# lbrndnr/LBAudioDetective

Measured on AMD Instinct MI355X. Metric: audio_seconds_fingerprinted_per_sec, higher is better.
Workload: dtype f32; 1 GPU; configs[1]: 100k synthetic 1 s @44.1 kHz mono clips, 1024-pt FFT, stride 64, fingerprint-only, input resident in HBM; one step = 13 passes over the batch; clips_per_gpu=100000, samples_per_clip=44100, window=1024, stride=64, bands=32, subfingerprints_per_clip=5, kernel_variant=0, parallelism=clips sharded x1, no collective

## Files before the change

### include/lbaudiodetective.h

```cpp
#ifndef LBAUDIODETECTIVE_H
#define LBAUDIODETECTIVE_H

#include <stddef.h>
#include <stdint.h>

#ifdef __cplusplus
extern "C" {
#endif

#if !defined(__MACTYPES__) && !defined(LBAD_HAVE_MACTYPES)
typedef uint32_t UInt32;
typedef int32_t SInt32;
typedef uint64_t UInt64;
typedef int64_t SInt64;
typedef float Float32;
typedef double Float64;
typedef unsigned char Boolean;
typedef SInt32 OSStatus;
enum { noErr = 0 };
#endif

#if !defined(__CoreAudioTypes_h__) && !defined(LBAD_HAVE_COREAUDIOTYPES)
typedef struct AudioStreamBasicDescription {
    Float64 mSampleRate;
// ... 115 lines not shown
                                                   UInt32 inResamplerMode, Float32** outSamples, UInt64* outCount,
                                                   Float64* outSampleRate);
void LBAudioDetectiveFreeSamples(Float32* inSamples);
OSStatus LBAudioDetectiveProcessFileStream(LBAudioDetectiveRef inDetective, const Float32* inClientSamples,
                                           UInt64 inClientCount, UInt64 inFileFrames, UInt32 inHop,
                                           LBAudioDetectiveFingerprintRef* outFingerprint);

UInt64 LBAudioDetectiveGetSubfingerprintCount(LBAudioDetectiveRef inDetective, UInt64 inNumberOfSamples);

OSStatus LBAudioDetectiveProcessPCM(LBAudioDetectiveRef inDetective, const Float32* inSamples,
                                    UInt64 inNumberOfSamples, LBAudioDetectiveFingerprintRef* outFingerprint);
OSStatus LBAudioDetectiveComparePCM(LBAudioDetectiveRef inDetective, const Float32* inSamples1, UInt64 inCount1,
                                    const Float32* inSamples2, UInt64 inCount2, UInt32 inComparisonRange,
                                    Float32* outMatch);

#define LBAD_PACKED_WORDS 8
#define LBAD_PACKED_BYTES 32
#define LBAD_MAX_SUBFINGERPRINT_LENGTH 256

OSStatus LBAudioDetectiveFingerprintClipsDevice(LBAudioDetectiveRef inDetective, const Float32* inClips,
                                                UInt64 inNumberOfClips, UInt64 inSamplesPerClip,
                                                void* outPacked, void* inStream);
OSStatus LBAudioDetectiveFingerprintClipsDeviceFormat(LBAudioDetectiveRef inDetective, const void* inClips,
                                                      UInt32 inSampleFormat, UInt64 inNumberOfClips,
                                                      UInt64 inSamplesPerClip, void* outPacked, void* inStream);
OSStatus LBAudioDetectiveFingerprintClips(LBAudioDetectiveRef inDetective, const Float32* inClips,
                                          UInt64 inNumberOfClips, UInt64 inSamplesPerClip, Boolean* outBooleans);
OSStatus LBAudioDetectiveFingerprintClipsFormat(LBAudioDetectiveRef inDetective, const void* inClips,
                                                UInt32 inSampleFormat, UInt64 inNumberOfClips,
                                                UInt64 inSamplesPerClip, Boolean* outBooleans);
OSStatus LBAudioDetectiveSetKernelVariant(LBAudioDetectiveRef inDetective, UInt32 inVariant);
OSStatus LBAudioDetectiveSetBandSumForm(LBAudioDetectiveRef inDetective, UInt32 inForm);
OSStatus LBAudioDetectiveGetBandSumForm(LBAudioDetectiveRef inDetective, UInt32* outForm);
OSStatus LBAudioDetectiveSetKernelTuning(LBAudioDetectiveRef inDetective, UInt32 inWavesPerWorkgroup,
                                         UInt32 inTwiddleCache);
OSStatus LBAudioDetectiveSetScratchLimit(LBAudioDetectiveRef inDetective, UInt64 inBytes);
OSStatus LBAudioDetectiveSetStageTiming(LBAudioDetectiveRef inDetective, UInt32 inEnabled);
OSStatus LBAudioDetectiveGetStageTimes(LBAudioDetectiveRef inDetective, Float32* outStage1Ms, Float32* outStage2Ms,
                                       UInt32* outLaunches);
OSStatus LBAudioDetectiveFingerprintClipsDeviceTaps(LBAudioDetectiveRef inDetective, const Float32* inClips,
                                                    UInt64 inNumberOfClips, UInt64 inSamplesPerClip,
                                                    void* outPacked, Float32* outFramesRaw, Float32* outFramesHaar,
                                                    void* inStream);
OSStatus LBAudioDetectiveFingerprintClipsDeviceTapsFormat(LBAudioDetectiveRef inDetective, const void* inClips,
                                                          UInt32 inSampleFormat, UInt64 inNumberOfClips,
                                                          UInt64 inSamplesPerClip, void* outPacked, Float32* outFramesRaw,
                                                          Float32* outFramesHaar, void* inStream);
OSStatus LBAudioDetectiveDebugStage1Choice(Float64 inSampleRate, UInt32 inWindowSize, UInt32 inAnalysisStride,
                                           UInt32 inNumberOfPitchSteps, UInt32 inSubfingerprintLength, UInt32 inKernelVariant,
                                           UInt32 inWavesPerWorkgroup, UInt32 inTwiddleCache, UInt32 inSampleFormat,
                                           UInt64 inNumberOfClips, UInt64 inSamplesPerClip, UInt32 inClipAddressMod8,
                                           UInt32 inRawTap, UInt32 inFileTail, UInt32* outWords, UInt32 inCapacity);

typedef struct LBAudioDetectiveStream* LBAudioDetectiveStreamRef;
LBAudioDetectiveStreamRef LBAudioDetectiveStreamNew(LBAudioDetectiveRef inDetective);
void LBAudioDetectiveStreamDispose(LBAudioDetectiveStreamRef inStream);
OSStatus LBAudioDetectiveStreamPush(LBAudioDetectiveStreamRef inStream, const Float32* inSamples,
                                    UInt64 inNumberOfSamples, UInt32* outNewSubfingerprints);
LBAudioDetectiveFingerprintRef LBAudioDetectiveStreamCopyFingerprint(LBAudioDetectiveStreamRef inStream);

typedef struct LBAudioDetectiveStreamBank* LBAudioDetectiveStreamBankRef;
LBAudioDetectiveStreamBankRef LBAudioDetectiveStreamBankNew(LBAudioDetectiveRef inDetective, UInt32 inNumberOfChannels,
                                                            UInt32 inHistorySubfingerprints, UInt32 inFramesPerPass);
void LBAudioDetectiveStreamBankDispose(LBAudioDetectiveStreamBankRef inBank);
OSStatus LBAudioDetectiveStreamBankPushDevice(LBAudioDetectiveStreamBankRef inBank, const Float32* inSamples,
                                              const UInt32* inSampleCounts, UInt32* outNewCounts, void* outNewPacked,
// ... 354 lines not shown
```

### lbaudiodetective_amd/_native.py

```python
from __future__ import annotations

import ctypes as C
import os
import subprocess

_HERE = os.path.dirname(os.path.abspath(__file__))
CSRC = os.path.join(_HERE, "csrc")
LIB_PATH = os.path.abspath(os.environ["LBAD_LIB"]) if os.environ.get("LBAD_LIB") else os.path.join(_HERE, "lib", "liblbaudiodetective.so")
HEADER = os.path.join(os.path.dirname(_HERE), "include", "lbaudiodetective.h")

UInt32, SInt32, UInt64, SInt64 = C.c_uint32, C.c_int32, C.c_uint64, C.c_int64
Float32, Float64, Boolean, OSStatus = C.c_float, C.c_double, C.c_ubyte, C.c_int32
Ref = C.c_void_p

PACKED_WORDS = 8
PACKED_BYTES = 32
SHARD_KEYS = 4096
ROWS_PER_FRAME = 128
SEGMENTS_MAX_SUBFINGERPRINTS = 8192


class AudioStreamBasicDescription(C.Structure):
    _fields_ = [
        ("mSampleRate", Float64), ("mFormatID", UInt32), ("mFormatFlags", UInt32),
# ... 82 lines not shown
    "LBAudioDetectiveCompactFramesToSubfingerprintsDevice": (OSStatus, [Ref, C.c_void_p, UInt64, C.c_void_p, C.c_void_p, C.c_void_p]),
    "LBAudioDetectiveFramesToSubfingerprintsDevice": (OSStatus, [Ref, C.c_void_p, UInt64, C.c_void_p, C.c_void_p, C.c_void_p]),
    "LBAudioDetectiveStreamNew": (Ref, [Ref]),
    "LBAudioDetectiveStreamDispose": (None, [Ref]),
    "LBAudioDetectiveStreamPush": (OSStatus, [Ref, C.c_void_p, UInt64, _P(UInt32)]),
    "LBAudioDetectiveStreamCopyFingerprint": (Ref, [Ref]),
    "LBAudioDetectiveStreamBankNew": (Ref, [Ref, UInt32, UInt32, UInt32]),
    "LBAudioDetectiveStreamBankDispose": (None, [Ref]),
    "LBAudioDetectiveStreamBankPushDevice": (OSStatus, [Ref, C.c_void_p, _P(UInt32), _P(UInt32), C.c_void_p, UInt64, _P(UInt64), C.c_void_p]),
    "LBAudioDetectiveStreamBankPush": (OSStatus, [Ref, C.c_void_p, _P(UInt32), _P(UInt32), C.c_void_p, UInt64, _P(UInt64), C.c_void_p]),
    "LBAudioDetectiveStreamBankGetCounts": (OSStatus, [Ref, _P(UInt64), _P(UInt32)]),
    "LBAudioDetectiveStreamBankWindowDevice": (OSStatus, [Ref, _P(UInt32), UInt32, UInt32, C.c_void_p, C.c_void_p]),
    "LBAudioDetectiveStreamBankCopyFingerprint": (Ref, [Ref, UInt32]),
    "LBAudioDetectiveStreamBankResetChannels": (OSStatus, [Ref, _P(UInt32), UInt32]),
    "LBAudioDetectiveDebugStreamBankPlan": (OSStatus, [UInt32, UInt32, UInt32, UInt32, _P(UInt32), _P(UInt32), _P(UInt32), _P(UInt32),
                                                       _P(UInt32)]),
    "LBAudioDetectiveResamplerBankNew": (Ref, [Float64, Float64, UInt32, UInt32]),
    "LBAudioDetectiveResamplerBankDispose": (None, [Ref]),
    "LBAudioDetectiveResamplerBankPushDevice": (OSStatus, [Ref, C.c_void_p, UInt32, _P(UInt32), _P(UInt32), C.c_void_p, UInt64, _P(UInt64),
                                                           C.c_void_p]),
    "LBAudioDetectiveResamplerBankPush": (OSStatus, [Ref, C.c_void_p, UInt32, _P(UInt32), _P(UInt32), C.c_void_p, UInt64, _P(UInt64),
                                                     C.c_void_p]),
    "LBAudioDetectiveResamplerBankFinishChannels": (OSStatus, [Ref, _P(UInt32), UInt32, _P(UInt32), C.c_void_p, UInt64, _P(UInt64),
                                                               C.c_void_p]),
    "LBAudioDetectiveResamplerBankGetCounts": (OSStatus, [Ref, _P(UInt64), _P(UInt64)]),
    "LBAudioDetectiveResamplerBankResetChannels": (OSStatus, [Ref, _P(UInt32), UInt32]),
    "LBAudioDetectiveDebugResamplerBankPlan": (OSStatus, [Float64, Float64, UInt32, UInt32, _P(UInt64), _P(UInt64), _P(UInt32), UInt32,
                                                          _P(UInt32), _P(UInt32), _P(SInt32), _P(SInt32)]),
    "LBAudioDetectiveFingerprintClips": (OSStatus, [Ref, C.c_void_p, UInt64, UInt64, C.c_void_p]),
    "LBAudioDetectiveFingerprintClipsFormat": (OSStatus, [Ref, C.c_void_p, UInt32, UInt64, UInt64, C.c_void_p]),
    "LBAudioDetectiveSetKernelVariant": (OSStatus, [Ref, UInt32]),
    "LBAudioDetectiveSetBandSumForm": (OSStatus, [Ref, UInt32]),
    "LBAudioDetectiveGetBandSumForm": (OSStatus, [Ref, _P(UInt32)]),
    "LBAudioDetectiveSetScratchLimit": (OSStatus, [Ref, UInt64]),
    "LBAudioDetectiveSetStageTiming": (OSStatus, [Ref, UInt32]),
    "LBAudioDetectiveGetStageTimes": (OSStatus, [Ref, _P(Float32), _P(Float32), _P(UInt32)]),
    "LBAudioDetectiveFingerprintClipsDeviceTapsFormat": (OSStatus, [Ref, C.c_void_p, UInt32, UInt64, UInt64, C.c_void_p, C.c_void_p,
                                                                    C.c_void_p, C.c_void_p]),
    "LBAudioDetectiveDebugStage1Choice": (OSStatus, [Float64, UInt32, UInt32, UInt32, UInt32, UInt32, UInt32, UInt32, UInt32, UInt64,
                                                     UInt64, UInt32, UInt32, UInt32, _P(UInt32), UInt32]),
    "LBAudioDetectiveFingerprintClipsDeviceTaps": (OSStatus, [Ref, C.c_void_p, UInt64, UInt64, C.c_void_p, C.c_void_p,
                                                              C.c_void_p, C.c_void_p]),
    "LBAudioDetectivePackSubfingerprint": (None, [C.c_void_p, UInt32, C.c_void_p]),
    "LBAudioDetectiveUnpackSubfingerprint": (None, [C.c_void_p, UInt32, C.c_void_p]),
    "LBAudioDetectiveCorpusNew": (Ref, [UInt32, UInt32, UInt64]),
    "LBAudioDetectiveCorpusNewRagged": (Ref, [UInt32, UInt64, UInt64]),
    "LBAudioDetectiveCorpusAppendRaggedPackedDevice": (OSStatus, [Ref, C.c_void_p, C.c_void_p, UInt64, C.c_void_p]),
    "LBAudioDetectiveCorpusGetSubfingerprintTotal": (UInt64, [Ref]),
    "LBAudioDetectiveSynthRaggedCorpusDevice": (OSStatus, [UInt32, UInt64, UInt64, C.c_void_p, UInt64, UInt32, C.c_void_p,
                                                           C.c_void_p]),
    "LBAudioDetectiveCorpusQuerySharded": (OSStatus, [Ref, Ref, UInt32, UInt64, C.c_void_p, C.c_void_p, _P(SInt64), _P(Float32)]),
    "LBAudioDetectiveCorpusQueryBatchSharded": (OSStatus, [Ref, _P(Ref), UInt32, UInt32, UInt64, C.c_void_p, C.c_void_p,
                                                           _P(SInt64), _P(Float32)]),
    "LBAudioDetectiveCorpusQueryBatchShardedWith": (OSStatus, [Ref, _P(Ref), UInt32, UInt32, UInt64, C.c_void_p, C.c_void_p,
                                                               C.c_void_p, _P(SInt64), _P(Float32)]),
    "LBAudioDetectiveSetExchangeTimeout": (None, [UInt32]),
    "LBAudioDetectiveCorpusSetBoundPruning": (OSStatus, [Ref, UInt32]),
    "LBAudioDetectiveCorpusSetBoundPruningThreshold": (OSStatus, [Ref, Float32]),
    "LBAudioDetectiveCorpusGetBoundPruningThreshold": (Float32, [Ref]),
    "LBAudioDetectiveCorpusShardKeysDevice": (C.c_void_p, [Ref]),
    "LBAudioDetectiveCorpusShardKeysHost": (C.c_void_p, [Ref]),
    "LBAudioDetectiveCommGetUniqueId": (OSStatus, [C.c_void_p]),
    "LBAudioDetectiveCommInitRank": (OSStatus, [_P(C.c_void_p), SInt32, C.c_void_p, SInt32]),
    "LBAudioDetectiveCommDestroy": (OSStatus, [C.c_void_p]),
    "LBAudioDetectiveCommGetInfo": (OSStatus, [C.c_void_p, _P(SInt32), _P(SInt32)]),
    "LBAudioDetectiveCorpusDispose": (None, [Ref]),
# ... 170 lines not shown
```

### lbaudiodetective_amd/csrc/api_detective.cpp

```cpp
#include "internal.hpp"
#include "const_div.hpp"

#include <new>
#include "audiofile.hpp"

#include <cmath>
#include <cstdlib>
#include <cstring>

namespace lbad {

uint64_t subfingerprint_count(uint64_t n_samples, uint32_t window, uint32_t stride) {
    if (stride == 0 || n_samples < window) return 0;
    return ((n_samples - window) / stride) / kRowsPerFrame;
}

static bool valid_window(uint32_t w) { return w >= kMinWindow && w <= kMaxWindow && (w & (w - 1)) == 0; }

static void free_plan(Plan& p) { p = Plan(); }

static void plan_kernels_host(Plan& p) {
    p.pruned_ok = rows_pruned_supported(p);
    p.lanes_ok = p.pruned_ok && rows_lanes_supported(p);
    p.full_ok = rows_full_supported(p);
// ... 485 lines not shown
}

OSStatus LBAudioDetectiveSetKernelVariant(LBAudioDetectiveRef d, UInt32 inVariant) {
    LBAD_LOCK(d);
    if (inVariant > 4) return kLBAudioDetectiveArgumentInvalid;
    d->variant = inVariant;
    return noErr;
}

static bool band_lanes_now(LBAudioDetectiveRef d) {
    lbad::Plan p;
    return lbad::plan_host(p, d->format.mSampleRate, d->window, d->stride, d->bands, d->subfp_len) == noErr && p.lanes_ok;
}

OSStatus LBAudioDetectiveSetBandSumForm(LBAudioDetectiveRef d, UInt32 inForm) {
    LBAD_GUARD_BEGIN
    LBAD_LOCK(d);
    if (!d || inForm > 2) return kLBAudioDetectiveArgumentInvalid;
    if (inForm == 2 && !band_lanes_now(d)) return kLBAudioDetectiveArgumentInvalid;
    d->band_form = inForm;
    return noErr;
    LBAD_GUARD_END
}

OSStatus LBAudioDetectiveGetBandSumForm(LBAudioDetectiveRef d, UInt32* outForm) {
    LBAD_GUARD_BEGIN
    LBAD_LOCK(d);
    if (!d || !outForm) return kLBAudioDetectiveArgumentInvalid;
    *outForm = d->band_form != 1 && band_lanes_now(d) ? 2u : 1u;
    return noErr;
    LBAD_GUARD_END
}

OSStatus LBAudioDetectiveSetKernelTuning(LBAudioDetectiveRef d, UInt32 inWavesPerWorkgroup, UInt32 inTwiddleCache) {
    LBAD_LOCK(d);
    if (!d || inWavesPerWorkgroup > 16) return kLBAudioDetectiveArgumentInvalid;
    d->tune_waves = inWavesPerWorkgroup;
    d->tune_cache = inTwiddleCache != 0;
    return noErr;
}

OSStatus LBAudioDetectiveSetScratchLimit(LBAudioDetectiveRef d, UInt64 inBytes) {
    LBAD_LOCK(d);
    if (!d || inBytes == 0) return kLBAudioDetectiveArgumentInvalid;
    d->scratch_limit = inBytes;
    return noErr;
}

OSStatus LBAudioDetectiveSetStageTiming(LBAudioDetectiveRef d, UInt32 inEnabled) {
    LBAD_LOCK(d);
    if (!d) return kLBAudioDetectiveArgumentInvalid;
    d->timing = inEnabled != 0;
    d->ev_used = 0;
    return noErr;
}

OSStatus LBAudioDetectiveGetStageTimes(LBAudioDetectiveRef d, Float32* outStage1Ms, Float32* outStage2Ms,
                                       UInt32* outLaunches) {
    LBAD_LOCK(d);
    if (!d || !d->timing || d->ev_used < 3) return kLBAudioDetectiveArgumentInvalid;
    float s1 = 0.0f, s2 = 0.0f;
    LBAD_HIP(hipEventSynchronize(d->ev[d->ev_used - 1]));
    for (size_t i = 0; i + 2 < d->ev_used; i += 3) {
        float a = 0.0f, b = 0.0f;
        LBAD_HIP(hipEventElapsedTime(&a, d->ev[i], d->ev[i + 1]));
        LBAD_HIP(hipEventElapsedTime(&b, d->ev[i + 1], d->ev[i + 2]));
// ... 511 lines not shown
```

### lbaudiodetective_amd/csrc/internal.hpp

```cpp
#pragma once

#include <hip/hip_runtime.h>

#include <algorithm>
#include <cstdint>
#include <cstdio>
#include <new>
#include <stdexcept>
#include <map>
#include <mutex>
#include <vector>

#include "../../include/lbaudiodetective.h"
#include "buffers.hpp"

namespace lbad {

constexpr uint32_t kRowsPerFrame = 128;
constexpr uint32_t kPackedWords = LBAD_PACKED_WORDS;
constexpr uint32_t kMaxBands = 64;
constexpr uint32_t kSparseFrameDwMax = 128 * 17;
constexpr uint32_t kMinWindow = 16;
constexpr uint32_t kMaxWindow = 8192;

// ... 69 lines not shown
        uint8_t pos_right[16];
        uint8_t pos_left = 0xFF;
        uint32_t frame_dw() const { return 128u * n_stored; }
    } sparse;
    uint32_t tune_waves = 0;
    bool tune_cache = true;
    bool valid = false;
};

struct FileDesc;
struct FileTail {
    uint32_t mode = 0;
    const FileDesc* d_files = nullptr;
    uint32_t n_files = 0;
    uint64_t max_rows = 0;
    uint64_t first_short = 0;
    uint64_t n_client = 0;
    const uint32_t* d_tbl = nullptr;
    uint64_t row_begin = 0;
    uint64_t rows = 0;
    uint64_t pcm_begin = 0;
};

hipError_t launch_fft_bands(const Plan& plan, const void* d_pcm, uint32_t fmt, uint64_t n_clips,
                            uint64_t samples_per_clip, uint32_t frames_per_clip, float* d_frames, hipStream_t stream);
hipError_t launch_haar_select(const Plan& plan, float* d_frames, uint64_t n_frames, uint32_t* d_packed,
                              float* d_haar_out, hipStream_t stream);
bool rows_pruned_supported(const Plan& plan);
void rows_pruned_constants(std::vector<float>& out);
hipError_t launch_rows_pruned(const Plan& plan, const float* d_bin_const, const void* d_pcm, uint32_t fmt,
                              uint64_t n_clips, uint64_t samples_per_clip, uint32_t frames_per_clip, float* d_frames,
                              hipStream_t stream, bool compact = false, uint32_t band_form = 0);
bool rows_lanes_supported(const Plan& plan);
void rows_lanes_table(const Plan& plan, std::vector<uint32_t>& band_tbl);

bool rows_full_supported(const Plan& plan);
bool rows_full_supported_fmt(const Plan& plan, uint32_t fmt);
hipError_t launch_rows_full(const Plan& plan, const void* d_pcm, uint32_t fmt, uint64_t n_clips,
                            uint64_t samples_per_clip, uint32_t frames_per_clip, float* d_frames, hipStream_t stream);

bool rows_stream_supported(const Plan& plan);
hipError_t launch_rows_stream(const Plan& plan, const void* d_pcm, uint32_t fmt, uint64_t n_clips,
                              uint64_t samples_per_clip, uint32_t frames_per_clip, float* d_frames, hipStream_t stream);

bool rows_stream2_supported(const Plan& plan);
hipError_t launch_rows_stream2(const Plan& plan, const void* d_pcm, uint32_t fmt, uint64_t n_clips,
                               uint64_t samples_per_clip, uint32_t frames_per_clip, float* d_frames, hipStream_t stream);

bool haar_select32_supported(const Plan& plan);
hipError_t launch_haar_select32(const Plan& plan, const float* d_frames, uint64_t n_frames, uint32_t* d_packed,
                                float* d_haar_out, hipStream_t stream, bool compact = false);
void plan_sparse(Plan& plan);

enum class Stage1Family : uint32_t { Generic = 0, Pruned = 1, Stream2 = 2, Full = 3, Stream = 4 };
struct FftBandsInstance {
    uint32_t log2w = 0, wpb = 0;
    bool cached = false;
};
FftBandsInstance fft_bands_instance(const Plan& plan);
struct RowsFullInstance {
    uint32_t log2l = 0, fmt = 0;
    bool s64 = false, lean = false, ok = false;
};
RowsFullInstance rows_full_instance(const Plan& plan, uint32_t fmt);
struct RowsStream2Instance {
    uint32_t fmt = 0, qlo = 0, qhi = 0;
// ... 670 lines not shown
```

### lbaudiodetective_amd/csrc/k_rows_pruned.hip

```cpp
#include "internal.hpp"

#include <cstring>
#include "const_div.hpp"
#include "fft64_lane.hpp"

namespace lbad {
namespace {

constexpr int kW = 1024;
constexpr int kStride = 64;
constexpr int kBands = 32;
constexpr int kBins = 22;
constexpr int kRows = 43;
constexpr int kRowsA = 22;
constexpr int kRowDw = 20;
constexpr int kWinDw = 464;
constexpr int kWaves = 4;
constexpr int kThreads = kWaves * 64;
constexpr int kUnitWindows = 32;
constexpr int kSpan = (kUnitWindows - 1) * kStride + kW;
constexpr int kSpanDw = kSpan + 16 * (kSpan >> 6);
constexpr int kTDw = kWaves * 8 * kWinDw;
constexpr int kBinConst = 14;
constexpr int kConstStride = 20;
// ... 352 lines not shown
        for (int rd = 0; rd < 3; ++rd)
            if (kLaneBin[j][rd] == k) return 8 * rd + j;
    return -1;
}
constexpr int lanes_band_of(int k) {
    for (int b = 0; b < kLaneBands; ++b)
        if (k >= kLaneBandLo[b] && k < kLaneBandHi[b]) return b;
    return -1;
}
constexpr uint32_t lanes_cont_mask(int rd) {
    uint32_t m = 0;
    for (int j = 0; j < 8; ++j)
        if (kLaneBin[j][rd] >= 0 && kLaneBin[j][rd] == kLaneBin[j][rd - 1] + 1 &&
            lanes_band_of(kLaneBin[j][rd]) == lanes_band_of(kLaneBin[j][rd - 1]))
            m |= 1u << j;
    return m;
}
constexpr uint64_t lanes_bin_pack(int rd) {
    uint64_t v = 0;
    for (int j = 0; j < 8; ++j) v |= (uint64_t)(kLaneBin[j][rd] >= 0 ? kLaneBin[j][rd] : 0) << (5 * j);
    return v;
}
constexpr bool lanes_table_ok() {
    for (int k = 0; k < kBins; ++k)
        if (lanes_pos(k) < 0 || lanes_pos(k) >= kBins || lanes_band_of(k) < 0) return false;
    for (int b = 0; b < kLaneBands; ++b) {
        for (int k = kLaneBandLo[b] + 1; k < kLaneBandHi[b]; ++k)
            if (lanes_pos(k) != lanes_pos(k - 1) + 8) return false;
    }
    return lanes_pos(kBins - 1) == kBins - 1;
}
static_assert(lanes_table_ok(), "every bin has one position below 22 and every band lies in one lane, in bin order");

template <int I, int END>
__device__ __forceinline__ void store_rows_lanes(const cplx (&x)[64], float* trow) {
    if constexpr (I < END) {
        *(lds_vf32x2*)(trow + lanes_pos(I) * kRowDw) = stage6_row<I>(x);
        store_rows_lanes<I + 1, END>(x, trow);
    }
}
template <int I, int N>
__device__ __forceinline__ void store_held_lanes(const cplx (&h)[kRows - kRowsA], float* trow) {
    if constexpr (I < N) {
        *(lds_vf32x2*)(trow + lanes_pos(kBins - 1 - I) * kRowDw) = h[I];
        store_held_lanes<I + 1, N>(h, trow);
    }
}

template <int FMT>
__global__ __launch_bounds__(kThreads, kWgPerCu) void frame_rows_lanes_kernel(const void* __restrict__ pcm_raw,
                                                                        uint64_t samples_per_clip,
                                                                        uint32_t frames_per_clip, uint64_t n_units,
                                                                        uint64_t units_per_xcd,
                                                                        const float* __restrict__ bin_const,
                                                                        const uint32_t* __restrict__ band_tbl,
                                                                        uint32_t* __restrict__ claim_ctr,
                                                                        float* __restrict__ frames, uint32_t frame_dw,
                                                                        uint32_t row_dw, uint32_t place_row) {
    extern __shared__ __attribute__((aligned(16))) float smem[];
    float* span = smem;
    const int wave = __builtin_amdgcn_readfirstlane(threadIdx.x >> 6);
    const int lane = threadIdx.x & 63;
    float* tbuf = smem + kSpanDw + wave * (8 * kWinDw);
    float* cbuf = smem + kSpanDw + kTDw;
    static_assert((kSpanDw + kTDw + kConstDw) % 2 == 0, "the slot behind the constants is 8-byte aligned");
    typedef __attribute__((address_space(3))) volatile uint64_t lds_vu64;
    lds_vu64* next_slot = (lds_vu64*)(cbuf + kConstDw);

    const uint32_t wg_per_xcd = gridDim.x >> 3;
    const uint64_t xcd_begin = (uint64_t)(blockIdx.x & 7) * units_per_xcd;
    const uint64_t xcd_end = xcd_begin + units_per_xcd < n_units ? xcd_begin + units_per_xcd : n_units;
    uint64_t unit = xcd_begin + 4 * (uint64_t)(blockIdx.x >> 3);
    if (unit >= xcd_end) {
        if (threadIdx.x == 0) claims_done(claim_ctr);
        return;
    }

    auto span_start = [&](uint64_t u) {
        const uint32_t frame = (uint32_t)(u >> 2);
        const uint32_t clip = frame / frames_per_clip;
        const uint32_t fi = frame - clip * frames_per_clip;
        return (uint64_t)clip * samples_per_clip + (uint64_t)(fi * 128 + (uint32_t)(u & 3) * kUnitWindows) * kStride;
    };
    uint32_t* my_ctr = claim_ctr + (blockIdx.x & 7);
    asm volatile("" : "+v"(my_ctr));
    const bool claimer = threadIdx.x == 0;
    uint32_t claimed = 0;
    uint64_t claim_base = xcd_begin + 4 * (uint64_t)wg_per_xcd;
    asm volatile("" : "+s"(claim_base));

    span_to_lds<FMT>(pcm_raw, span_start(unit), span, wave, lane);
    for (int i = threadIdx.x; i < kBins * kBinConst; i += kThreads) {
        const int p = i / kBinConst;
        constexpr uint64_t kBin0 = lanes_bin_pack(0), kBin1 = lanes_bin_pack(1), kBin2 = lanes_bin_pack(2);
        const int k = (int)(((p < 8 ? kBin0 : p < 16 ? kBin1 : kBin2) >> (5 * (p & 7))) & 31u);
        cbuf[p * kConstStride + (i % kBinConst)] = bin_const[k * kBinConst + (i % kBinConst)];
    }

    const int w8 = lane >> 3, r = lane & 7;
    const float inv_norm = 1.0f / (float)(kW / 4);
    const int rr = r ^ ((((w8 + 1) >> 1) & 1) << 2);
    int tk[3];
#pragma unroll
    for (int rd = 0; rd < 3; ++rd) tk[rd] = rr + 8 * rd < kBins ? rr + 8 * rd : kBins - 1;

    const uint32_t* task_tbl = band_tbl + kLanesFirstRow * kBands;
    float t_div[3], t_rcp[3];
    uint32_t t_off = 0, z_off = 0;
    bool proven = true;
#pragma unroll
    for (int rd = 0; rd < 3; ++rd) {
        t_div[rd] = __uint_as_float(task_tbl[8 * rd + rr]);
        t_rcp[rd] = __uint_as_float(task_tbl[kBands + 8 * rd + rr]);
        proven = proven && task_tbl[2 * kBands + 8 * rd + rr] != 0u;
        t_off |= (task_tbl[place_row * kBands + 8 * rd + rr] & 0xFFu) << (8 * rd);
        z_off |= (task_tbl[5 * kBands + 8 * rd + rr] & 0xFFu) << (8 * rd);
    }
    const int t_fast_hi = proven ? (int)kBandDivHi : -1;
    constexpr uint32_t kCont1 = lanes_cont_mask(1), kCont2 = lanes_cont_mask(2);
    const uint32_t m_cont1 = (kCont1 >> rr) & 1u ? 0xFFFFFFFFu : 0u;
    const uint32_t m_cont2 = (kCont2 >> rr) & 1u ? 0xFFFFFFFFu : 0u;
    const bool is_dc = rr == 0;

    __syncthreads();
    TreeTw twp[3], twm[3];
    f32x2 ws[3];
#pragma unroll
    for (int rd = 0; rd < 3; ++rd) {
        const float* c = cbuf + tk[rd] * kConstStride;
        twp[rd] = tree_twiddles(c);
        twm[rd] = tree_twiddles(c + 6);
        ws[rd] = *reinterpret_cast<const f32x2*>(c + 12);
    }

    float out[3] = {0.0f, 0.0f, 0.0f};
    float* out_row = nullptr;
#ifdef LBAD_EXP_TIMELINE
    long long ts[8];
#define STAMP(i) ts[i] = __builtin_readcyclecounter()
#else
#define STAMP(i)
#endif
    auto store_out = [&]() {
        if (!out_row) return;
        uint32_t places = t_off;
        asm volatile("" : "+v"(places));
#pragma unroll
        for (int rd = 0; rd < 3; ++rd) {
            const uint32_t o = (places >> (8 * rd)) & 0xFFu;
            if (o != 0xFFu) out_row[o] = out[rd];
        }
        uint32_t layout = place_row;
        asm volatile("" : "+s"(layout));
        if (layout == 3u) {
            places = z_off;
            asm volatile("" : "+v"(places));
#pragma unroll
            for (int rd = 0; rd < 3; ++rd) {
                const uint32_t o = (places >> (8 * rd)) & 0xFFu;
                if (o != 0xFFu) out_row[o] = 0.0f;
            }
        }
    };
    for (;;) {
        STAMP(0);
#ifdef LBAD_EXP_TIMELINE
        const unsigned long long rt0 = __builtin_amdgcn_s_memrealtime();
#endif
        __builtin_amdgcn_s_waitcnt(0x0F70);
        const uint32_t quarter = (uint32_t)(unit & 3);
        if (quarter == 3 && claimer) *next_slot = claim_base + 4 * (uint64_t)claimed;
        __syncthreads();
        STAMP(1);

        cplx x[64];
        load_points<0>(x, span + 80 * (8 * wave + w8) + 2 * r);
        const uint64_t next = quarter == 3 ? *next_slot : unit + 1;
        __syncthreads();
        if (next < xcd_end) span_to_lds<FMT>(pcm_raw, span_start(next), span, wave, lane);
        if (quarter == 0 && claimer) claimed = atomicAdd(my_ctr, 1u);
#ifndef LBAD_EXP_TIMELINE
        store_out();
#endif
        STAMP(2);

        __builtin_amdgcn_s_setprio(0);
        stage_blocks<1, 0>(x);
        stage_blocks<2, 0>(x);
        stage_blocks<3, 0>(x);
        stage_blocks<4, 0>(x);
        stage_blocks<5, 0>(x);
        STAMP(3);
        __builtin_amdgcn_s_setprio(3);

        store_rows_lanes<0, kRowsA>(x, tbuf + w8 * kWinDw + 2 * r);
        cplx held[kRows - kRowsA];
        hold_rows<kRowsA, kRows, kRowsA>(x, held);
        cplx za[3];
        {
            TreeIn in[3];
#pragma unroll
            for (int rd = 0; rd < 3; ++rd) in[rd] = tree_load(tbuf + w8 * kWinDw + tk[rd] * kRowDw);
            store_held_lanes<0, kRows - kRowsA>(held, tbuf + w8 * kWinDw + 2 * r);
#pragma unroll
            for (int rd = 0; rd < 3; ++rd) za[rd] = tree_eval(in[rd], twp[rd]);
        }
        STAMP(4);
        float pw[3];
        {
            TreeIn in[3];
#pragma unroll
            for (int rd = 0; rd < 3; ++rd) in[rd] = tree_load(tbuf + w8 * kWinDw + tk[rd] * kRowDw);
#pragma unroll
            for (int rd = 0; rd < 3; ++rd) {
                const cplx b = tree_eval(in[rd], twm[rd]);
                const cplx a = za[rd];
                float re, im;
                if (rd == 0 && is_dc) {
                    const float sm = a.x + a.y, df = a.x - a.y;
                    re = sm + sm;
                    im = df + df;
                } else {
                    const float sr = a.x + b.x, si = a.y - b.y;
                    const float dr = a.x - b.x, di = a.y + b.y;
                    const float wr = ws[rd].x, wi = ws[rd].y;
                    re = __fmaf_rn(wr, di, __fmaf_rn(wi, dr, sr));
                    im = __fmaf_rn(-wr, dr, __fmaf_rn(wi, di, si));
                }
                if (re > 0.0f) re = __fmul_rn(re, inv_norm);
                if (im > 0.0f) im = __fmul_rn(im, inv_norm);
                pw[rd] = __fadd_rn(__fmul_rn(re, re), __fmul_rn(im, im));
            }
        }
        STAMP(5);

        float s[3];
#pragma unroll
        for (int rd = 0; rd < 3; ++rd) s[rd] = pw[rd] < INFINITY ? pw[rd] : 0.0f;
        s[1] = __fadd_rn(__uint_as_float(__float_as_uint(s[0]) & m_cont1), s[1]);
        s[2] = __fadd_rn(__uint_as_float(__float_as_uint(s[1]) & m_cont2), s[2]);
        DivGuard g;
        g.dividends(s[0], s[1]);
        g.dividends(s[2], s[2]);
        const int s_max = max(max((int)__float_as_uint(s[0]), (int)__float_as_uint(s[1])), (int)__float_as_uint(s[2]));
        if (__builtin_expect(__builtin_amdgcn_ballot_w64(g.lo < 2u * kBandDivLo - 1u || s_max > t_fast_hi) == 0, 1)) {
#pragma unroll
            for (int rd = 0; rd < 3; ++rd) out[rd] = div_c<true>(s[rd], t_div[rd], t_rcp[rd]);
        } else {
#pragma unroll
            for (int rd = 0; rd < 3; ++rd) out[rd] = div_c<false>(s[rd], t_div[rd], t_rcp[rd]);
        }
        out_row = frames + (unit >> 2) * frame_dw + (quarter * kUnitWindows + 8 * wave + w8) * row_dw;
#ifdef LBAD_EXP_TIMELINE
        asm volatile("" ::"v"(out[0]), "v"(out[1]), "v"(out[2]));
        STAMP(6);
        if (lane == 0) {
            float* o = frames + ((unit >> 2) * 128 + quarter * kUnitWindows + 8 * wave) * kBands;
            for (int i = 1; i < 7; ++i) o[i - 1] = (float)(ts[i] - ts[i - 1]);
            o[6] = (float)(ts[0] & 0xFFFFFF);
            o[7] = (float)__builtin_amdgcn_s_getreg(((16 - 1) << 11) | 4);
            o[8] = (float)(ts[0] >> 24 & 0xFFFFFF);
            o[9] = (float)(__builtin_amdgcn_s_memrealtime() - rt0);
        }
#endif
        if (next >= xcd_end) break;
        unit = next;
    }
#ifndef LBAD_EXP_TIMELINE
    store_out();
#endif
    if (claimer) claims_done(claim_ctr);
}
#undef STAMP

}

bool rows_pruned_supported(const Plan& p) {
    if (p.window != (uint32_t)kW || p.stride != (uint32_t)kStride || p.bands != (uint32_t)kBands) return false;
    if (p.table.kmax > (uint32_t)kBins) return false;
    std::vector<float> re, im;
    make_twiddles(kW, re, im);
    for (int t = 0; t < 32; ++t)
        if (re[16 * t] != kTw64Re[t] || im[16 * t] != kTw64Im[t]) return false;
    return true;
}

void rows_pruned_constants(std::vector<float>& out) {
    std::vector<float> re, im;
    make_twiddles(kW, re, im);
    out.assign((size_t)kClaimOffset + kClaimWords, 0.0f);
    for (int k = 0; k < kBins; ++k) {
        float* c = &out[(size_t)k * kBinConst];
        c[0] = re[8 * k]; c[1] = im[8 * k];
        c[2] = re[4 * k]; c[3] = im[4 * k];
        c[4] = re[2 * k]; c[5] = im[2 * k];
        if (k > 0) {
            c[6] = -re[8 * (64 - k)];   c[7] = -im[8 * (64 - k)];
            c[8] = -re[4 * (128 - k)];  c[9] = -im[4 * (128 - k)];
            c[10] = -re[2 * (256 - k)]; c[11] = -im[2 * (256 - k)];
            c[12] = re[k]; c[13] = im[k];
        }
    }
}

// ... 30 lines not shown
    for (uint32_t b = 0; b < (uint32_t)kBands; ++b) {
        if (p.table.lo[b] >= p.table.hi[b]) {
            if (empty < 24) t[5 * kBands + empty] = b;
            ++empty;
            continue;
        }
        const float div = (float)(p.table.indices[b + 1] - p.table.indices[b]);
        const float rcp = 1.0f / div;
        for (uint32_t k = p.table.lo[b]; k < p.table.hi[b]; ++k) {
            const int at = lanes_pos((int)k);
            std::memcpy(&t[at], &div, 4);
            std::memcpy(&t[kBands + at], &rcp, 4);
            t[2 * kBands + at] = band_div_proven(div) ? 1u : 0u;
            if (k + 1 != p.table.hi[b]) continue;
            t[3 * kBands + at] = b;
            if (p.sparse.ok) {
                const uint32_t pos = b >= 16 ? p.sparse.pos_right[b - 16] : (b == p.sparse.left ? p.sparse.pos_left : 0xFFu);
                if (pos != 0xFFu) t[4 * kBands + at] = pos;
            }
        }
    }
}

template <int FMT>
static hipError_t launch_rows_fmt(const Plan& plan, const float* d_bin_const, const void* d_pcm, uint64_t n_frames,
                                  uint64_t samples_per_clip, uint32_t frames_per_clip, float* d_frames,
                                  hipStream_t stream, bool compact, bool lanes) {
    static PerDevice attr, attr_lanes;
    if (!lanes && attr.changed(kLdsBytes)) {
        hipError_t e = hipFuncSetAttribute(reinterpret_cast<const void*>(frame_rows_pruned_kernel<FMT>),
                                           hipFuncAttributeMaxDynamicSharedMemorySize, kLdsBytes);
        if (e != hipSuccess) return e;
    }
    if (lanes && attr_lanes.changed(kLdsBytes)) {
        hipError_t e = hipFuncSetAttribute(reinterpret_cast<const void*>(frame_rows_lanes_kernel<FMT>),
                                           hipFuncAttributeMaxDynamicSharedMemorySize, kLdsBytes);
        if (e != hipSuccess) return e;
    }
    const uint64_t n_units = n_frames * 4, units_per_xcd = 4 * ((n_frames + 7) / 8);
    const int n_cu = device_cu_count();
    uint64_t wg_per_xcd = ((uint64_t)n_cu * kWgPerCu + 7) / 8;
    if (wg_per_xcd > units_per_xcd / 4) wg_per_xcd = units_per_xcd / 4;
    uint32_t* claim = reinterpret_cast<uint32_t*>(const_cast<float*>(d_bin_const)) + kClaimOffset;
    if (lanes)
        hipLaunchKernelGGL(frame_rows_lanes_kernel<FMT>, dim3((uint32_t)(wg_per_xcd * 8)), dim3(kThreads), kLdsBytes,
                           stream, d_pcm, samples_per_clip, frames_per_clip, n_units, units_per_xcd, d_bin_const,
                           plan.d_bands, claim, d_frames, compact ? plan.sparse.frame_dw() : 128u * kBands,
                           compact ? plan.sparse.n_stored : (uint32_t)kBands, compact ? 4u : 3u);
    else
        hipLaunchKernelGGL(frame_rows_pruned_kernel<FMT>, dim3((uint32_t)(wg_per_xcd * 8)), dim3(kThreads), kLdsBytes,
                           stream, d_pcm, samples_per_clip, frames_per_clip, n_units, units_per_xcd, d_bin_const,
                           plan.d_bands, claim, d_frames, compact ? plan.sparse.frame_dw() : 128u * kBands, compact ? 5u : 3u);
    return hipGetLastError();
}

hipError_t launch_rows_pruned(const Plan& plan, const float* d_bin_const, const void* d_pcm, uint32_t fmt,
                              uint64_t n_clips, uint64_t samples_per_clip, uint32_t frames_per_clip, float* d_frames,
                              hipStream_t stream, bool compact, uint32_t band_form) {
    if (compact && !plan.sparse.ok) return hipErrorInvalidValue;
    if (band_form > 2 || (band_form == 2 && !plan.lanes_ok)) return hipErrorInvalidValue;
    const bool lanes = band_form != 1 && plan.lanes_ok;
    const uint64_t n_frames = n_clips * frames_per_clip;
    if (n_frames == 0) return hipSuccess;
    if (n_frames > 0x7fffffffull) return hipErrorInvalidValue;
    if (n_frames * 4 + 8 > 0x7fffffffull) return hipErrorInvalidValue;
    switch (fmt) {
        case 0: return launch_rows_fmt<0>(plan, d_bin_const, d_pcm, n_frames, samples_per_clip, frames_per_clip, d_frames, stream, compact, lanes);
        case 1: return launch_rows_fmt<1>(plan, d_bin_const, d_pcm, n_frames, samples_per_clip, frames_per_clip, d_frames, stream, compact, lanes);
        case 2: return launch_rows_fmt<2>(plan, d_bin_const, d_pcm, n_frames, samples_per_clip, frames_per_clip, d_frames, stream, compact, lanes);
        default: return hipErrorInvalidValue;
    }
}

}
```

Before: 5.687 million audio-s/s.

## Double-buffer PCM spans and swizzle transpose layout in lanes row kernel

Measured after the change: 5.604 million audio-s/s. -1.5%, worse.

```diff
diff --git a/include/lbaudiodetective.h b/include/lbaudiodetective.h
--- a/include/lbaudiodetective.h
+++ b/include/lbaudiodetective.h
@@ -171,6 +171,7 @@
 OSStatus LBAudioDetectiveSetKernelVariant(LBAudioDetectiveRef inDetective, UInt32 inVariant);
 OSStatus LBAudioDetectiveSetBandSumForm(LBAudioDetectiveRef inDetective, UInt32 inForm);
 OSStatus LBAudioDetectiveGetBandSumForm(LBAudioDetectiveRef inDetective, UInt32* outForm);
+UInt32 LBAudioDetectiveDebugBandSumFormLdsBytes(UInt32 inForm);
 OSStatus LBAudioDetectiveSetKernelTuning(LBAudioDetectiveRef inDetective, UInt32 inWavesPerWorkgroup,
                                          UInt32 inTwiddleCache);
 OSStatus LBAudioDetectiveSetScratchLimit(LBAudioDetectiveRef inDetective, UInt64 inBytes);
diff --git a/lbaudiodetective_amd/_native.py b/lbaudiodetective_amd/_native.py
--- a/lbaudiodetective_amd/_native.py
+++ b/lbaudiodetective_amd/_native.py
@@ -138,6 +138,7 @@
     "LBAudioDetectiveSetKernelVariant": (OSStatus, [Ref, UInt32]),
     "LBAudioDetectiveSetBandSumForm": (OSStatus, [Ref, UInt32]),
     "LBAudioDetectiveGetBandSumForm": (OSStatus, [Ref, _P(UInt32)]),
+    "LBAudioDetectiveDebugBandSumFormLdsBytes": (UInt32, [UInt32]),
     "LBAudioDetectiveSetScratchLimit": (OSStatus, [Ref, UInt64]),
     "LBAudioDetectiveSetStageTiming": (OSStatus, [Ref, UInt32]),
     "LBAudioDetectiveGetStageTimes": (OSStatus, [Ref, _P(Float32), _P(Float32), _P(UInt32)]),
diff --git a/lbaudiodetective_amd/csrc/api_detective.cpp b/lbaudiodetective_amd/csrc/api_detective.cpp
--- a/lbaudiodetective_amd/csrc/api_detective.cpp
+++ b/lbaudiodetective_amd/csrc/api_detective.cpp
@@ -541,6 +541,8 @@
     LBAD_GUARD_END
 }
 
+UInt32 LBAudioDetectiveDebugBandSumFormLdsBytes(UInt32 inForm) { return lbad::rows_pruned_lds_bytes(inForm); }
+
 OSStatus LBAudioDetectiveSetKernelTuning(LBAudioDetectiveRef d, UInt32 inWavesPerWorkgroup, UInt32 inTwiddleCache) {
     LBAD_LOCK(d);
     if (!d || inWavesPerWorkgroup > 16) return kLBAudioDetectiveArgumentInvalid;
diff --git a/lbaudiodetective_amd/csrc/internal.hpp b/lbaudiodetective_amd/csrc/internal.hpp
--- a/lbaudiodetective_amd/csrc/internal.hpp
+++ b/lbaudiodetective_amd/csrc/internal.hpp
@@ -125,6 +125,7 @@
                               uint64_t n_clips, uint64_t samples_per_clip, uint32_t frames_per_clip, float* d_frames,
                               hipStream_t stream, bool compact = false, uint32_t band_form = 0);
 bool rows_lanes_supported(const Plan& plan);
+uint32_t rows_pruned_lds_bytes(uint32_t band_form);
 void rows_lanes_table(const Plan& plan, std::vector<uint32_t>& band_tbl);
 
 bool rows_full_supported(const Plan& plan);
diff --git a/lbaudiodetective_amd/csrc/k_rows_pruned.hip b/lbaudiodetective_amd/csrc/k_rows_pruned.hip
--- a/lbaudiodetective_amd/csrc/k_rows_pruned.hip
+++ b/lbaudiodetective_amd/csrc/k_rows_pruned.hip
@@ -408,18 +408,145 @@
 }
 static_assert(lanes_table_ok(), "every bin has one position below 22 and every band lies in one lane, in bin order");
 
+constexpr int kLRowDw = 16;
+constexpr int kLWinDw = 368;
+constexpr int kLTDw = kWaves * 8 * kLWinDw;
+constexpr int kLTreeBase = 2 * kSpanDw;
+constexpr int kLanesLdsBytes = (2 * kSpanDw + kLTDw + kConstDw + 4) * 4;
+static_assert(kWgPerCu * kLanesLdsBytes <= 160 * 1024, "two workgroups must fit one CU's LDS");
+static_assert(kLWinDw >= kBins * kLRowDw && kLWinDw <= 391, "22 rows fit a window, and 32 windows fit beside two spans");
+
+constexpr int lanes_rot(int w8) { return w8 & 3; }
+constexpr int lanes_rr(int w8, int r) { return r ^ ((((w8 + 1) >> 1) & 1) << 2); }
+constexpr int lanes_write_dw(int w8, int r, int pos) { return w8 * kLWinDw + pos * kLRowDw + ((2 * r + 4 * lanes_rot(w8)) & 15); }
+constexpr int lanes_read_dw(int w8, int r, int rd, int c) {
+    const int j = lanes_rr(w8, r) + 8 * rd;
+    return w8 * kLWinDw + (j < kBins ? j : kBins - 1) * kLRowDw + 4 * ((c + lanes_rot(w8)) & 3);
+}
+constexpr bool lanes_layout_ok() {
+    for (int g = 0; g < 4; ++g)
+        for (int pos = 0; pos < kBins; ++pos) {
+            int hits[32] = {};
+            for (int lane = 16 * g; lane < 16 * g + 16; ++lane) {
+                const int a = kLTreeBase + lanes_write_dw(lane >> 3, lane & 7, pos);
+                if (a % 2 != 0) return false;
+                ++hits[a % 32];
+                ++hits[(a + 1) % 32];
+            }
+            for (int b = 0; b < 32; ++b)
+                if (hits[b] != 1) return false;
+        }
+    for (int half = 0; half < 2; ++half)
+        for (int grp = 0; grp < 2; ++grp) {
+            int lanes[16] = {};
+            for (int i = 0; i < 4; ++i) lanes[i] = 32 * half + (grp ? 4 : 0) + i;
+            for (int i = 0; i < 4; ++i) lanes[4 + i] = 32 * half + (grp ? 8 : 12) + i;
+            for (int i = 0; i < 4; ++i) lanes[8 + i] = 32 * half + (grp ? 16 : 20) + i;
+            for (int i = 0; i < 4; ++i) lanes[12 + i] = 32 * half + (grp ? 28 : 24) + i;
+            for (int rd = 0; rd < 3; ++rd)
+                for (int c = 0; c < 4; ++c)
+                    for (int i = 0; i < 16; ++i)
+                        for (int k = i + 1; k < 16; ++k) {
+                            const int a = kLTreeBase + lanes_read_dw(lanes[i] >> 3, lanes[i] & 7, rd, c);
+                            const int b = kLTreeBase + lanes_read_dw(lanes[k] >> 3, lanes[k] & 7, rd, c);
+                            if (a % 4 != 0 || b % 4 != 0) return false;
+                            if (a != b && (a / 4) % 16 == (b / 4) % 16) return false;
+                        }
+        }
+    for (int w8 = 0; w8 < 8; ++w8)
+        for (int r = 0; r < 8; ++r)
+            for (int rd = 0; rd < 3; ++rd) {
+                const int j = lanes_rr(w8, r) + 8 * rd;
+                if (j >= kBins) continue;
+                for (int s = 0; s < 8; ++s)
+                    if (lanes_write_dw(w8, s, j) != lanes_read_dw(w8, r, rd, s >> 1) + 2 * (s & 1)) return false;
+            }
+    return true;
+}
+static_assert(lanes_layout_ok(), "the transpose image of frame_rows_lanes_kernel: conflict-free stores and tree reads");
+
 template <int I, int END>
 __device__ __forceinline__ void store_rows_lanes(const cplx (&x)[64], float* trow) {
     if constexpr (I < END) {
-        *(lds_vf32x2*)(trow + lanes_pos(I) * kRowDw) = stage6_row<I>(x);
+        *(lds_vf32x2*)(trow + lanes_pos(I) * kLRowDw) = stage6_row<I>(x);
         store_rows_lanes<I + 1, END>(x, trow);
     }
 }
 template <int I, int N>
 __device__ __forceinline__ void store_held_lanes(const cplx (&h)[kRows - kRowsA], float* trow) {
     if constexpr (I < N) {
-        *(lds_vf32x2*)(trow + lanes_pos(kBins - 1 - I) * kRowDw) = h[I];
+        *(lds_vf32x2*)(trow + lanes_pos(kBins - 1 - I) * kLRowDw) = h[I];
         store_held_lanes<I + 1, N>(h, trow);
+    }
+}
+__device__ __forceinline__ TreeIn tree_load_rot(const float* s0, const float* s1, const float* s2, const float* s3) {
+    TreeIn in;
+    in.q0 = *reinterpret_cast<const float4*>(s0);
+    in.q1 = *reinterpret_cast<const float4*>(s1);
+    in.q2 = *reinterpret_cast<const float4*>(s2);
+    in.q3 = *reinterpret_cast<const float4*>(s3);
+    return in;
+}
+
+template <int FMT>
+__device__ __forceinline__ void span_to_buffer(const void* __restrict__ pcm_raw, uint64_t first, float* span, int wave,
+                                            int lane) {
+    if constexpr (FMT == 0) {
+        const uint64_t first_w = first + 64 * wave;
+        const uint64_t first_s = ((uint64_t)__builtin_amdgcn_readfirstlane((uint32_t)(first_w >> 32)) << 32) |
+                                 (uint32_t)__builtin_amdgcn_readfirstlane((uint32_t)first_w);
+        const char* src = static_cast<const char*>(pcm_raw) + 4 * first_s;
+        const uint32_t lane_off = 4u * (uint32_t)lane;
+        uint32_t lbase = (uint32_t)(size_t)(lvoid_t*)(span + 80 * wave);
+        int tail_wave = wave;
+        asm volatile("" : "+s"(lbase), "+s"(tail_wave));
+        constexpr int kFull = (kSpan / 64) / kWaves;
+        static_assert(kFull == 11, "three groups of four loads");
+#define LBAD_SPAN_LOAD(I)                                                                                            \
+    __builtin_amdgcn_global_load_lds((gvoid_t*)(src + 4 * 64 * kWaves * ((I) & ~3) + lane_off),                      \
+                                     (lvoid_t*)(size_t)(lbase + 4 * (80 * kWaves * (I) - 64 * kWaves * ((I) & 3))),  \
+                                     4, 4 * 64 * kWaves * ((I) & 3), 0)
+        LBAD_SPAN_LOAD(0); LBAD_SPAN_LOAD(1); LBAD_SPAN_LOAD(2); LBAD_SPAN_LOAD(3);
+        LBAD_SPAN_LOAD(4); LBAD_SPAN_LOAD(5); LBAD_SPAN_LOAD(6); LBAD_SPAN_LOAD(7);
+        LBAD_SPAN_LOAD(8); LBAD_SPAN_LOAD(9); LBAD_SPAN_LOAD(10);
+        if (tail_wave < kSpan / 64 - kFull * kWaves) LBAD_SPAN_LOAD(11);
+#undef LBAD_SPAN_LOAD
+    } else if constexpr (FMT == 1) {
+        const int16_t* src = static_cast<const int16_t*>(pcm_raw) + first;
+        for (int s = threadIdx.x; s < kSpan; s += kThreads)
+            span[s + 16 * (s >> 6)] = (float)src[s] * (1.0f / 32768.0f);
+    } else {
+        const int32_t* src = static_cast<const int32_t*>(pcm_raw) + first;
+        for (int s = threadIdx.x; s < kSpan; s += kThreads)
+            span[s + 16 * (s >> 6)] = (float)src[s] * (1.0f / 2147483648.0f);
+    }
+}
+
+template <int G>
+__device__ __forceinline__ void load_point_group(cplx (&x)[64], const float* src) {
+    if constexpr (G < 8) {
+#pragma unroll
+        for (int i = 0; i < 8; ++i) {
+            const int m = brev6(8 * G + i);
+            x[8 * G + i] = *(const lds_vf32x2*)(src + (m & 3) * 16 + (m >> 2) * 80);
+        }
+    }
+}
+template <int G>
+__device__ __forceinline__ void points_and_first_stages(cplx (&x)[64], const float* src) {
+    if constexpr (G < 8) {
+        load_point_group<G + 2>(x, src);
+        stage_block_j<1, 8 * G, 0>(x);
+        stage_block_j<1, 8 * G + 2, 0>(x);
+        stage_block_j<1, 8 * G + 4, 0>(x);
+        stage_block_j<1, 8 * G + 6, 0>(x);
+        stage_block_j<2, 8 * G, 0>(x);
+        stage_block_j<2, 8 * G + 4, 0>(x);
+        stage_block_j<3, 8 * G, 0>(x);
+#pragma unroll
+        for (int i = 0; i < 8; ++i) asm volatile("" ::"v"(x[8 * G + i]));
+        __builtin_amdgcn_sched_barrier(0);
+        points_and_first_stages<G + 1>(x, src);
     }
 }
 
@@ -433,13 +560,14 @@
                                                                         uint32_t* __restrict__ claim_ctr,
                                                                         float* __restrict__ frames, uint32_t frame_dw,
                                                                         uint32_t row_dw, uint32_t place_row) {
-    extern __shared__ __attribute__((aligned(16))) float smem[];
+    extern __shared__ __attribute__((aligned(16))) float smem_lanes[];
+    float* const smem = smem_lanes;
     float* span = smem;
     const int wave = __builtin_amdgcn_readfirstlane(threadIdx.x >> 6);
     const int lane = threadIdx.x & 63;
-    float* tbuf = smem + kSpanDw + wave * (8 * kWinDw);
-    float* cbuf = smem + kSpanDw + kTDw;
-    static_assert((kSpanDw + kTDw + kConstDw) % 2 == 0, "the slot behind the constants is 8-byte aligned");
+    float* tbuf = smem + kLTreeBase + wave * (8 * kLWinDw);
+    float* cbuf = smem + kLTreeBase + kLTDw;
+    static_assert((kLTreeBase + kLTDw + kConstDw) % 2 == 0, "the slot behind the constants is 8-byte aligned");
     typedef __attribute__((address_space(3))) volatile uint64_t lds_vu64;
     lds_vu64* next_slot = (lds_vu64*)(cbuf + kConstDw);
 
@@ -460,12 +588,17 @@
     };
     uint32_t* my_ctr = claim_ctr + (blockIdx.x & 7);
     asm volatile("" : "+v"(my_ctr));
-    const bool claimer = threadIdx.x == 0;
+    uint32_t tid = threadIdx.x;
+    auto claimer = [&]() {
+        uint32_t t = tid;
+        asm volatile("" : "+v"(t));
+        return t == 0;
+    };
     uint32_t claimed = 0;
-    uint64_t claim_base = xcd_begin + 4 * (uint64_t)wg_per_xcd;
-    asm volatile("" : "+s"(claim_base));
-
-    span_to_lds<FMT>(pcm_raw, span_start(unit), span, wave, lane);
+    if (threadIdx.x == 0) next_slot[1] = xcd_begin + 4 * (uint64_t)wg_per_xcd;
+
+    span_to_buffer<FMT>(pcm_raw, span_start(unit), span, wave, lane);
+    span_to_buffer<FMT>(pcm_raw, span_start(unit + 1), span + kSpanDw, wave, lane);
     for (int i = threadIdx.x; i < kBins * kBinConst; i += kThreads) {
         const int p = i / kBinConst;
         constexpr uint64_t kBin0 = lanes_bin_pack(0), kBin1 = lanes_bin_pack(1), kBin2 = lanes_bin_pack(2);
@@ -497,7 +630,16 @@
     const uint32_t m_cont1 = (kCont1 >> rr) & 1u ? 0xFFFFFFFFu : 0u;
     const uint32_t m_cont2 = (kCont2 >> rr) & 1u ? 0xFFFFFFFFu : 0u;
     const bool is_dc = rr == 0;
-
+    float* trow = tbuf + w8 * kLWinDw + ((2 * r + 4 * lanes_rot(w8)) & 15);
+    const float* s_lo[4];
+    const float* s_hi[4];
+#pragma unroll
+    for (int c = 0; c < 4; ++c) {
+        s_lo[c] = tbuf + w8 * kLWinDw + rr * kLRowDw + 4 * ((c + lanes_rot(w8)) & 3);
+        s_hi[c] = s_lo[c] + (tk[2] - rr) * kLRowDw;
+    }
+
+    __builtin_amdgcn_s_waitcnt(0x0F70);
     __syncthreads();
     TreeTw twp[3], twm[3];
     f32x2 ws[3];
@@ -543,41 +685,50 @@
 #ifdef LBAD_EXP_TIMELINE
         const unsigned long long rt0 = __builtin_amdgcn_s_memrealtime();
 #endif
+        const uint32_t quarter = (uint32_t)(unit & 3);
+        float* buf = span + (quarter & 1u) * kSpanDw;
+        if (quarter == 2 && claimer()) next_slot[0] = next_slot[1] + 4 * (uint64_t)claimed;
+        STAMP(1);
+        cplx x[64];
+        {
+            const float* src = buf + 80 * (8 * wave + w8) + 2 * r;
+            load_point_group<0>(x, src);
+            load_point_group<1>(x, src);
+            __builtin_amdgcn_sched_barrier(0);
+            points_and_first_stages<0>(x, src);
+        }
+
         __builtin_amdgcn_s_waitcnt(0x0F70);
-        const uint32_t quarter = (uint32_t)(unit & 3);
-        if (quarter == 3 && claimer) *next_slot = claim_base + 4 * (uint64_t)claimed;
         __syncthreads();
-        STAMP(1);
-
-        cplx x[64];
-        load_points<0>(x, span + 80 * (8 * wave + w8) + 2 * r);
-        const uint64_t next = quarter == 3 ? *next_slot : unit + 1;
-        __syncthreads();
-        if (next < xcd_end) span_to_lds<FMT>(pcm_raw, span_start(next), span, wave, lane);
-        if (quarter == 0 && claimer) claimed = atomicAdd(my_ctr, 1u);
+        __builtin_amdgcn_sched_barrier(0);
+        const uint64_t claimed_unit = quarter >= 2 ? next_slot[0] : 0;
+        const uint64_t next = quarter == 3 ? claimed_unit : unit + 1;
+        const uint32_t next2 = quarter >= 2 ? (uint32_t)claimed_unit + (quarter - 2) : (uint32_t)unit + 2;
+        if (next2 < (uint32_t)xcd_end) span_to_buffer<FMT>(pcm_raw, span_start(next2), buf, wave, lane);
+        if (quarter == 0 && claimer()) claimed = atomicAdd(my_ctr, 1u);
 #ifndef LBAD_EXP_TIMELINE
         store_out();
 #endif
         STAMP(2);
 
         __builtin_amdgcn_s_setprio(0);
-        stage_blocks<1, 0>(x);
-        stage_blocks<2, 0>(x);
-        stage_blocks<3, 0>(x);
         stage_blocks<4, 0>(x);
         stage_blocks<5, 0>(x);
         STAMP(3);
         __builtin_amdgcn_s_setprio(3);
 
-        store_rows_lanes<0, kRowsA>(x, tbuf + w8 * kWinDw + 2 * r);
+        store_rows_lanes<0, kRowsA>(x, trow);
         cplx held[kRows - kRowsA];
         hold_rows<kRowsA, kRows, kRowsA>(x, held);
         cplx za[3];
         {
             TreeIn in[3];
 #pragma unroll
-            for (int rd = 0; rd < 3; ++rd) in[rd] = tree_load(tbuf + w8 * kWinDw + tk[rd] * kRowDw);
-            store_held_lanes<0, kRows - kRowsA>(held, tbuf + w8 * kWinDw + 2 * r);
+            for (int rd = 0; rd < 2; ++rd)
+                in[rd] = tree_load_rot(s_lo[0] + 8 * rd * kLRowDw, s_lo[1] + 8 * rd * kLRowDw, s_lo[2] + 8 * rd * kLRowDw,
+                                       s_lo[3] + 8 * rd * kLRowDw);
+            in[2] = tree_load_rot(s_hi[0], s_hi[1], s_hi[2], s_hi[3]);
+            store_held_lanes<0, kRows - kRowsA>(held, trow);
 #pragma unroll
             for (int rd = 0; rd < 3; ++rd) za[rd] = tree_eval(in[rd], twp[rd]);
         }
@@ -586,7 +737,10 @@
         {
             TreeIn in[3];
 #pragma unroll
-            for (int rd = 0; rd < 3; ++rd) in[rd] = tree_load(tbuf + w8 * kWinDw + tk[rd] * kRowDw);
+            for (int rd = 0; rd < 2; ++rd)
+                in[rd] = tree_load_rot(s_lo[0] + 8 * rd * kLRowDw, s_lo[1] + 8 * rd * kLRowDw, s_lo[2] + 8 * rd * kLRowDw,
+                                       s_lo[3] + 8 * rd * kLRowDw);
+            in[2] = tree_load_rot(s_hi[0], s_hi[1], s_hi[2], s_hi[3]);
 #pragma unroll
             for (int rd = 0; rd < 3; ++rd) {
                 const cplx b = tree_eval(in[rd], twm[rd]);
@@ -645,7 +799,7 @@
 #ifndef LBAD_EXP_TIMELINE
     store_out();
 #endif
-    if (claimer) claims_done(claim_ctr);
+    if (threadIdx.x == 0) claims_done(claim_ctr);
 }
 #undef STAMP
 
@@ -742,9 +896,9 @@
                                            hipFuncAttributeMaxDynamicSharedMemorySize, kLdsBytes);
         if (e != hipSuccess) return e;
     }
-    if (lanes && attr_lanes.changed(kLdsBytes)) {
+    if (lanes && attr_lanes.changed(kLanesLdsBytes)) {
         hipError_t e = hipFuncSetAttribute(reinterpret_cast<const void*>(frame_rows_lanes_kernel<FMT>),
-                                           hipFuncAttributeMaxDynamicSharedMemorySize, kLdsBytes);
+                                           hipFuncAttributeMaxDynamicSharedMemorySize, kLanesLdsBytes);
         if (e != hipSuccess) return e;
     }
     const uint64_t n_units = n_frames * 4, units_per_xcd = 4 * ((n_frames + 7) / 8);
@@ -753,7 +907,7 @@
     if (wg_per_xcd > units_per_xcd / 4) wg_per_xcd = units_per_xcd / 4;
     uint32_t* claim = reinterpret_cast<uint32_t*>(const_cast<float*>(d_bin_const)) + kClaimOffset;
     if (lanes)
-        hipLaunchKernelGGL(frame_rows_lanes_kernel<FMT>, dim3((uint32_t)(wg_per_xcd * 8)), dim3(kThreads), kLdsBytes,
+        hipLaunchKernelGGL(frame_rows_lanes_kernel<FMT>, dim3((uint32_t)(wg_per_xcd * 8)), dim3(kThreads), kLanesLdsBytes,
                            stream, d_pcm, samples_per_clip, frames_per_clip, n_units, units_per_xcd, d_bin_const,
                            plan.d_bands, claim, d_frames, compact ? plan.sparse.frame_dw() : 128u * kBands,
                            compact ? plan.sparse.n_stored : (uint32_t)kBands, compact ? 4u : 3u);
@@ -762,6 +916,10 @@
                            stream, d_pcm, samples_per_clip, frames_per_clip, n_units, units_per_xcd, d_bin_const,
                            plan.d_bands, claim, d_frames, compact ? plan.sparse.frame_dw() : 128u * kBands, compact ? 5u : 3u);
     return hipGetLastError();
+}
+
+uint32_t rows_pruned_lds_bytes(uint32_t band_form) {
+    return band_form == 2 ? (uint32_t)kLanesLdsBytes : band_form == 1 ? (uint32_t)kLdsBytes : 0u;
 }
 
 hipError_t launch_rows_pruned(const Plan& plan, const float* d_bin_const, const void* d_pcm, uint32_t fmt,
```
